# louiskirsch/speechT

Hardware: AMD Instinct MI355X
Metric: utterances/sec (training step, 10 s@16 kHz, batch 32) (higher is better)
Workload: dtype f32

## Files before the change

speecht_amd/csrc/api.hip:

```cpp
#include <algorithm>
#include <atomic>
#include <mutex>
#include <string>
#include <vector>
#include <string.h>

#include "st_common.h"

namespace st {
static thread_local char g_err[512] = "";
void set_error(const char* fmt, ...) {
  va_list ap;
  va_start(ap, fmt);
  vsnprintf(g_err, sizeof(g_err), fmt, ap);
  va_end(ap);
}

static std::atomic<int> g_trace_on{0};
static std::mutex g_trace_mu;
static std::vector<std::string> g_lines;
constexpr int kMaxTimed = 1 << 14;
struct TimedLaunch { int line; hipEvent_t e0, e1; };
static std::vector<TimedLaunch> g_timed;
static thread_local int g_last_line = -1;
static std::string g_timed_filter;
bool trace_on() { return g_trace_on.load(std::memory_order_relaxed) != 0; }
void trace(const char* fmt, ...) {
  if (!trace_on()) return;
  char line[320];
  va_list ap;
  va_start(ap, fmt);
  vsnprintf(line, sizeof(line), fmt, ap);
  va_end(ap);
  std::lock_guard<std::mutex> lock(g_trace_mu);
  if (g_lines.size() < (1u << 16)) {
    g_last_line = (int)g_lines.size();
    g_lines.emplace_back(line);
  } else {
    g_last_line = -1;
  }
}
LaunchTimer::LaunchTimer(hipStream_t) : start_(nullptr), stop_(nullptr) {
  const int line = g_last_line;
  g_last_line = -1;
  if (g_trace_on.load(std::memory_order_relaxed) != 2 || line < 0) return;
  hipEvent_t e0 = nullptr, e1 = nullptr;
  if (hipEventCreate(&e0) != hipSuccess) return;
  if (hipEventCreate(&e1) != hipSuccess) { hipEventDestroy(e0); return; }
  std::lock_guard<std::mutex> lock(g_trace_mu);
  if ((int)g_timed.size() >= kMaxTimed || line >= (int)g_lines.size() ||
      (!g_timed_filter.empty() && g_lines[line].find(g_timed_filter) == std::string::npos)) {
    hipEventDestroy(e0);
    hipEventDestroy(e1);
    return;
  }
  g_timed.push_back(TimedLaunch{line, e0, e1});
  start_ = e0;
  stop_ = e1;
}

static const char* const kTuneNames[TUNE_COUNT] = {"streamk", "streamk_slots", "streamk_test_drop", "no_fused_transforms",
                                                   "bf16_lag_copies", "filters_idft_valu", "bf16_taps_panel", "no_g3", "g3_tile"};
static std::atomic<int> g_tune[TUNE_COUNT];
int tuning(int key) { return g_tune[key].load(std::memory_order_relaxed); }
}

extern "C" {
int st_version(void) { return 200; }
const char* st_last_error(void) { return st::g_err; }

static int trace_begin(int mode) {
  std::lock_guard<std::mutex> lock(st::g_trace_mu);
  st::g_lines.clear();
  for (auto& t : st::g_timed) { hipEventDestroy(t.e0); hipEventDestroy(t.e1); }
  st::g_timed.clear();
  st::g_last_line = -1;
  st::g_trace_on.store(mode);
  return ST_OK;
}
int st_trace_begin(void) { return trace_begin(1); }
int st_trace_begin_timed(void) { return trace_begin(2); }
int st_trace_timed_filter(const char* text) {
  std::lock_guard<std::mutex> lock(st::g_trace_mu);
  st::g_timed_filter = text ? text : "";
  return ST_OK;
}

size_t st_trace_end(char* host_buf, size_t capacity) {
  st::g_trace_on.store(0);
  std::lock_guard<std::mutex> lock(st::g_trace_mu);
  for (auto& t : st::g_timed) {
    float ms = -1.f;
    if (hipEventSynchronize(t.e1) != hipSuccess || hipEventElapsedTime(&ms, t.e0, t.e1) != hipSuccess) ms = -1.f;
    char tail[48];
    snprintf(tail, sizeof(tail), " ms=%.5f", ms);
    if (t.line >= 0 && t.line < (int)st::g_lines.size()) st::g_lines[t.line] += tail;
    hipEventDestroy(t.e0);
    hipEventDestroy(t.e1);
  }
  st::g_timed.clear();
  size_t need = 1;
  for (const auto& l : st::g_lines) need += l.size() + 1;
  if (host_buf && capacity > 0) {
    size_t at = 0;
    for (const auto& l : st::g_lines) {
      if (at + l.size() + 1 >= capacity) break;
      memcpy(host_buf + at, l.data(), l.size());
      at += l.size();
      host_buf[at++] = '\n';
    }
    host_buf[at] = 0;
  }
  return need;
}

uint32_t st_host_crc32c(const void* host_data, size_t n, uint32_t crc) {
  static uint32_t table[8][256];
  static std::once_flag once;
  std::call_once(once, [] {
    for (uint32_t i = 0; i < 256; ++i) {
      uint32_t c = i;
      for (int k = 0; k < 8; ++k) c = (c >> 1) ^ (0x82F63B78u & (0u - (c & 1u)));
      table[0][i] = c;
    }
    for (uint32_t i = 0; i < 256; ++i)
      for (int t = 1; t < 8; ++t) table[t][i] = (table[t - 1][i] >> 8) ^ table[0][table[t - 1][i] & 0xFF];
  });
  const unsigned char* p = reinterpret_cast<const unsigned char*>(host_data);
  crc = ~crc;
  while (n >= 8) {
    uint32_t lo, hi;
    memcpy(&lo, p, 4);
    memcpy(&hi, p + 4, 4);
    lo ^= crc;
    crc = table[7][lo & 0xFF] ^ table[6][(lo >> 8) & 0xFF] ^ table[5][(lo >> 16) & 0xFF] ^ table[4][lo >> 24] ^
          table[3][hi & 0xFF] ^ table[2][(hi >> 8) & 0xFF] ^ table[1][(hi >> 16) & 0xFF] ^ table[0][hi >> 24];
    p += 8;
    n -= 8;
  }
  while (n--) crc = (crc >> 8) ^ table[0][(crc ^ *p++) & 0xFF];
  return ~crc;
}

int st_set_tuning(const char* name, int value) {
  ST_REQUIRE(name, "st_set_tuning: null name");
// ... 10 lines not shown
```

speecht_amd/csrc/conv_gemm.hip:

```cpp
#include <algorithm>
#include <atomic>
#include <cmath>
#include <cstdlib>

#include <type_traits>

#include "st_common.h"
#include "streamk_map.h"

namespace {

typedef float f32x16 __attribute__((ext_vector_type(16)));
typedef float f32x4 __attribute__((ext_vector_type(4)));

constexpr int BK = 32;
constexpr int APITCH = BK + 4;
constexpr int NTHREADS = 256;

struct RowMap {
  int frames;
  int row_stride;
  long batch_stride;
  long row0;
  __device__ __forceinline__ long off(int m) const {
    int b = m / frames;
    int t = m - b * frames;
    return (long)b * batch_stride + row0 + (long)t * row_stride;
  }
};

struct NNParams {
  const float* A;  RowMap amap;
  const float* Bm; int Np;
  float* C;        RowMap cmap;
  const float* mask; RowMap mmap;
  const float* bias;
  int M, Kvalid, Kp, n_store, relu;
  int taps, cp;
  int tiles_m, tiles_n, chunk;
  int gm, tm_per, tn_per;
  int splits, steps_per_split;
  float* slab;
  float* colsum;
  int colsum_rows;
  int batches;
  long a_batch, b_batch, c_batch;
  long bt_ld; int bt_rows;
};


__device__ __forceinline__ void dma16_sv(unsigned lds_byte_addr, const void* sbase, unsigned voff_bytes) {
  unsigned keep;
  asm volatile("s_mov_b32 %0, m0\n\ts_mov_b32 m0, %1\n\ts_nop 0\n\tglobal_load_lds_dwordx4 %2, %3\n\ts_mov_b32 m0, %0"
               : "=&s"(keep) : "s"(lds_byte_addr), "v"(voff_bytes), "s"(sbase) : "memory");
}
__device__ __forceinline__ float* at_bytes(float* ubase, unsigned voff_bytes) {
  return reinterpret_cast<float*>(reinterpret_cast<char*>(ubase) + voff_bytes);
}
__device__ __forceinline__ const float* at_bytes(const float* ubase, unsigned voff_bytes) {
  return reinterpret_cast<const float*>(reinterpret_cast<const char*>(ubase) + voff_bytes);
}
__device__ __forceinline__ void dma_wait_all() { asm volatile("s_waitcnt vmcnt(0)" ::: "memory"); }
__device__ __forceinline__ unsigned lds_addr(const float* p) {
  return (unsigned)(size_t)(__attribute__((address_space(3))) const float*)p;
}

template <int N> struct FVec;
template <> struct FVec<1> { typedef float type; };
template <> struct FVec<2> { typedef float type __attribute__((ext_vector_type(2))); };
template <> struct FVec<4> { typedef float type __attribute__((ext_vector_type(4))); };
template <int N> __device__ __forceinline__ float vget(const typename FVec<N>::type& v, int i) { return v[i]; }
template <> __device__ __forceinline__ float vget<1>(const float& v, int) { return v; }
template <int N> __device__ __forceinline__ void vset(typename FVec<N>::type& v, int i, float x) { v[i] = x; }
template <> __device__ __forceinline__ void vset<1>(float& v, int, float x) { v = x; }

__device__ __forceinline__ int swz_slot4(int lane, int row) { return ((lane & 7) ^ ((row >> 1) & 7)) * 4; }
__device__ __forceinline__ int swz_frag(int row, int q, int h) { return row * BK + (((2 * q + h) ^ ((row >> 1) & 7)) * 4); }

template <int BM, int BN, int WMW, int WNW, bool BT>
struct NNStage {
  static constexpr int WTM = BM / WMW, WTN = BN / WNW;
  static constexpr int MT = WTM / 32, NT = WTN / 32;
  static constexpr int A_DMA = BM / 32;
  static constexpr int B_DMA = BN / 32;
  static constexpr int N_DMA = A_DMA + B_DMA;
  static constexpr int A_SZ = BM * BK, B_SZ = BK * BN;
  typedef typename FVec<NT>::type bvec;

  template <int CUR, bool MORE, typename Dma, typename... Next>
  static __device__ __forceinline__ void run(const float* As, const float* Bs, const int (&a_frag)[4], const int (&bt_frag)[4],
                                             int b_frag, f32x16 (&acc)[MT][NT], int nq, Dma& dma_piece, Next... next) {
    const float* as = As + CUR * A_SZ;
    const float* bs = Bs + CUR * B_SZ + (BT ? 0 : b_frag);
    f32x4 af[4][MT];
    bvec bf[4][4];
    f32x4 bft[4][NT];
    auto read_frags = [&](int q) {
#pragma unroll
      for (int i = 0; i < MT; ++i) af[q][i] = *reinterpret_cast<const f32x4*>(as + a_frag[q] + i * 32 * BK);
      if (BT) {
#pragma unroll
        for (int n = 0; n < NT; ++n) bft[q][n] = *reinterpret_cast<const f32x4*>(bs + bt_frag[q] + n * 32 * BK);
      } else {
#pragma unroll
        for (int j = 0; j < 4; ++j) bf[q][j] = *reinterpret_cast<const bvec*>(bs + (8 * q + j) * BN);
      }
    };
    read_frags(0);
#pragma unroll
    for (int q = 0; q < 4; ++q) {
      if (MORE) {
#pragma unroll
        for (int pc = q; pc < N_DMA; pc += 4) dma_piece(pc, next..., CUR ^ 1);
      }
      if (q < 3) read_frags(q + 1);
      if (q < nq) {
#pragma unroll
        for (int j = 0; j < 4; ++j)
#pragma unroll
          for (int i = 0; i < MT; ++i)
#pragma unroll
            for (int n = 0; n < NT; ++n)
              acc[i][n] = __builtin_amdgcn_mfma_f32_32x32x2f32(af[q][i][j], BT ? bft[q][n][j] : vget<NT>(bf[q][j], n), acc[i][n], 0, 0, 0);
      }
#pragma unroll
      for (int k = 0; k < 4; ++k) {
        __builtin_amdgcn_sched_group_barrier(0x008, 1, 0);
        __builtin_amdgcn_sched_group_barrier(0x100, 1, 0);
      }
#pragma unroll
      for (int k = 0; k < 2; ++k) {
        __builtin_amdgcn_sched_group_barrier(0x008, 2, 0);
        __builtin_amdgcn_sched_group_barrier(0x006, 8, 0);
        __builtin_amdgcn_sched_group_barrier(0x010, 1, 0);
      }
      __builtin_amdgcn_sched_group_barrier(0x008, 8, 0);
      __builtin_amdgcn_sched_barrier(0);
// ... 556 lines not shown
    const int row = wn * WTN + l31;
#pragma unroll
    for (int q = 0; q < 4; ++q) bt_frag[q] = swz_frag(row, q, h);
  }
  const int b_frag = (4 * h) * BN + wn * WTN + NT * l31;

  f32x16 acc[MT][NT] = {}, acc2[MT][NT];

#pragma unroll
  for (int pcx = 0; pcx < N_DMA; ++pcx) dma_piece(pcx, p.a_off[0], p.b_off[0], 0);
  __syncthreads();

  auto stage = [&](auto cur_c, auto more_c, f32x16 (&tgt)[MT][NT], long nao, long nbo) __attribute__((always_inline)) {
    S::template run<decltype(cur_c)::value, decltype(more_c)::value>(As, Bs, a_frag, bt_frag, b_frag, tgt, 4, dma_piece, nao, nbo);
  };
  using std::integral_constant;
  using std::true_type;
  using std::false_type;
  const int spp = p.K / BK;
  auto phase = [&](f32x16 (&tgt)[MT][NT], long ao, long bo, long next_ao, long next_bo, auto last_c) __attribute__((always_inline)) {
    constexpr bool LAST = decltype(last_c)::value;
    for (int kt = 0; kt + 2 < spp; kt += 2) {
      stage(integral_constant<int, 0>{}, true_type{}, tgt, ao + (kt + 1) * BK, bo + (kt + 1) * bstep);
      stage(integral_constant<int, 1>{}, true_type{}, tgt, ao + (kt + 2) * BK, bo + (kt + 2) * bstep);
    }
    stage(integral_constant<int, 0>{}, true_type{}, tgt, ao + (spp - 1) * BK, bo + (spp - 1) * bstep);
    if (LAST) stage(integral_constant<int, 1>{}, false_type{}, tgt, 0L, 0L);
    else stage(integral_constant<int, 1>{}, true_type{}, tgt, next_ao, next_bo);
  };
  phase(acc, p.a_off[0], p.b_off[0], p.a_off[1], p.b_off[1], false_type{});
#pragma unroll
  for (int i = 0; i < MT; ++i)
#pragma unroll
    for (int j = 0; j < NT; ++j) acc2[i][j] = acc[i][j];
  phase(acc, p.a_off[1], p.b_off[1], p.a_off[2], p.b_off[2], false_type{});
  phase(acc2, p.a_off[2], p.b_off[2], 0L, 0L, true_type{});

  float* __restrict__ Cb = p.C + (long)bin * p.c_batch + n0 + wn * WTN + (BT ? l31 : NT * l31);
#pragma unroll
  for (int i = 0; i < MT; ++i)
#pragma unroll
    for (int r = 0; r < 16; ++r) {
      const int m = m0 + wm * WTM + i * 32 + (r & 3) + 8 * (r >> 2) + 4 * h;
      if (m < p.M) {
        float* row = Cb + (long)m * p.ldc;
        if (p.ksplit > 1) {
#pragma unroll
          for (int n = 0; n < NT; ++n) {
            const int cn = BT ? n * 32 : n;
            __hip_atomic_fetch_add(row + cn, acc[i][n][r], __ATOMIC_RELAXED, __HIP_MEMORY_SCOPE_AGENT);
            __hip_atomic_fetch_add(row + p.c_off2 + cn, acc2[i][n][r], __ATOMIC_RELAXED, __HIP_MEMORY_SCOPE_AGENT);
          }
        } else if (BT) {
#pragma unroll
          for (int n = 0; n < NT; ++n) { row[n * 32] = acc[i][n][r]; row[p.c_off2 + n * 32] = acc2[i][n][r]; }
        } else {
          bvec o1, o2;
#pragma unroll
          for (int n = 0; n < NT; ++n) { vset<NT>(o1, n, acc[i][n][r]); vset<NT>(o2, n, acc2[i][n][r]); }
          *reinterpret_cast<bvec*>(row) = o1;
          *reinterpret_cast<bvec*>(row + p.c_off2) = o2;
        }
      }
    }
}

struct TNParams {
  const float* A; RowMap amap;
  const float* Z; RowMap zmap;
  float* out;
  int M, Kvalid, Kp, Np, z_cols;
  int rows_per_split;
  int tiles_k, tiles_n;
  int amap_batches;
  int adv_b, adv_t;
  long a_batch, z_batch, o_batch;
  int z_shift;
};

__device__ __attribute__((aligned(16))) float g_zero_row[4] = {0.f, 0.f, 0.f, 0.f};

constexpr int TN_THREADS = NTHREADS;

template <int BN, int WKW, int WNW>
__global__ __launch_bounds__(TN_THREADS) void gemm_tn_kernel(TNParams p) {
  constexpr int BKO = 128;
  constexpr int BMR = 32;
  constexpr int WTK = BKO / WKW, WTN = BN / WNW;
  constexpr int MT = WTK / 32, NT = WTN / 32;
  constexpr int A_DMA = BKO / 32, Z_DMA = BN / 32;
  constexpr int A_LPR = BKO / 4, Z_LPR = BN / 4;
  constexpr int A_SZ = BMR * BKO, Z_SZ = BMR * BN;
  constexpr int N_DMA = A_DMA + Z_DMA;
  static_assert(WKW * WNW == 4 && (MT == 1 || MT == 2 || MT == 4) && (NT == 1 || NT == 2 || NT == 4), "tile config");
  typedef typename FVec<MT>::type avec;
  typedef typename FVec<NT>::type zvec;

  __shared__ __attribute__((aligned(16))) float smem[2 * A_SZ + 2 * Z_SZ];
  float* const As = smem;
  float* const Zs = smem + 2 * A_SZ;

  int tile_k, tile_n;
  {
    const int bid = blockIdx.x;
    const int total = p.tiles_k * p.tiles_n;
    if ((p.tiles_k & 7) == 0 && (p.tiles_n & 7) == 0) {
      const int idx = (bid & 7) * (total >> 3) + (bid >> 3);
      const int sb = idx >> 6, within = idx & 63;
      const int sbn = p.tiles_n >> 3;
      tile_k = (sb / sbn) * 8 + (within >> 3);
      tile_n = (sb % sbn) * 8 + (within & 7);
    } else {
      tile_n = bid % p.tiles_n;
      tile_k = bid / p.tiles_n;
    }
  }
  const int k0 = tile_k * BKO, n0 = tile_n * BN;
  const int split = blockIdx.y;
  const float* __restrict__ Ab = p.A + (long)blockIdx.z * p.a_batch;
  const float* __restrict__ Zb = p.Z + (long)(blockIdx.z >> p.z_shift) * p.z_batch;
  const int m_begin = split * p.rows_per_split;
  const int m_end = min(p.M, m_begin + p.rows_per_split);

  const int tid = threadIdx.x;
  const int lane = tid & 63;
  const int wave = __builtin_amdgcn_readfirstlane(tid >> 6);
  const int l31 = lane & 31, h = lane >> 5;
  const int wk = wave / WNW, wn = wave % WNW;

  f32x16 acc[MT][NT] = {};

  const int nstages = (m_end - m_begin + BMR - 1) / BMR;

  constexpr int A_PIECES = BMR * A_LPR / 64, Z_PIECES = BMR * Z_LPR / 64;
  constexpr int A_PW = (A_PIECES + 3) / 4, Z_PW = (Z_PIECES + 3) / 4;
  const int acol = min(k0 + (lane % A_LPR) * 4, p.Kvalid - 4);
  const int zcol = min(n0 + (lane % Z_LPR) * 4, p.z_cols - 4);
  const int arow = lane / A_LPR, zrow = lane / Z_LPR;
  const long a_jump = p.amap.batch_stride - (long)p.amap.frames * p.amap.row_stride;
  const long z_jump = p.zmap.batch_stride - (long)p.zmap.frames * p.zmap.row_stride;
  const bool tiny = p.amap.frames < BMR;
  const unsigned a_voff = (unsigned)((arow * p.amap.row_stride + acol) * 4);
  const unsigned z_voff = (unsigned)((zrow * p.zmap.row_stride + zcol) * 4);
  const unsigned lds_a = lds_addr(As), lds_z = lds_addr(Zs);
  const long a_step = (long)(64 / A_LPR) * p.amap.row_stride * 4, z_step = (long)(64 / Z_LPR) * p.zmap.row_stride * 4;
  int sb = min(m_begin, p.M - 1) / p.amap.frames;
  int stt = min(m_begin, p.M - 1) - sb * p.amap.frames;

  auto issue_slice = [&](int sl, int mb, int buf) {
    const bool plain = !tiny && stt + BMR <= p.amap.frames && mb + BMR <= m_end;
    if (plain) {
      const char* sa = reinterpret_cast<const char*>(Ab + ((long)sb * p.amap.batch_stride + p.amap.row0 + (long)stt * p.amap.row_stride));
      const char* sz = reinterpret_cast<const char*>(Zb + ((long)sb * p.zmap.batch_stride + p.zmap.row0 + (long)stt * p.zmap.row_stride));
#pragma unroll
      for (int i = sl; i < A_PW; i += 4) {
        const int pc = wave * A_PW + i;
        if (pc < A_PIECES) dma16_sv(lds_a + (buf * A_SZ + pc * 256) * 4, sa + pc * a_step, a_voff);
      }
#pragma unroll
      for (int i = sl; i < Z_PW; i += 4) {
        const int pc = wave * Z_PW + i;
        if (pc < Z_PIECES) dma16_sv(lds_z + (buf * Z_SZ + pc * 256) * 4, sz + pc * z_step, z_voff);
      }
    } else {
#pragma unroll
      for (int i = sl; i < A_PW + Z_PW; i += 4) {
        const bool isA = i < A_PW;
        const int pc = isA ? wave * A_PW + i : wave * Z_PW + (i - A_PW);
        if (pc >= (isA ? A_PIECES : Z_PIECES)) continue;
        const int r = isA ? pc * (64 / A_LPR) + arow : pc * (64 / Z_LPR) + zrow;
        const int m = min(mb + r, p.M - 1);
        const float* g = isA ? Ab + p.amap.off(m) + acol : Zb + p.zmap.off(m) + zcol;
        if (mb + r >= m_end) g = g_zero_row;
        float* dst = isA ? As + buf * A_SZ + pc * 256 : Zs + buf * Z_SZ + pc * 256;
        __builtin_amdgcn_global_load_lds((st::gptr_t)g, (st::lptr_t)dst, 16, 0, 0);
      }
    }
  };
  auto stage_advance = [&]() {
    stt += p.adv_t; sb += p.adv_b;
    if (stt >= p.amap.frames) { stt -= p.amap.frames; ++sb; }
  };

  if (nstages > 0) {
#pragma unroll
    for (int sl = 0; sl < 4; ++sl) issue_slice(sl, m_begin, 0);
    stage_advance();
  }
  dma_wait_all();
  __syncthreads();

  const int a_frag = (4 * h) * BKO + wk * WTK + MT * l31;
  const int z_frag = (4 * h) * BN + wn * WTN + NT * l31;
  for (int st = 0; st < nstages; ++st) {
    const int cur = st & 1;
    const bool more = st + 1 < nstages;
    const int mb_next = m_begin + (st + 1) * BMR;
    const float* as = As + cur * A_SZ + a_frag;
    const float* zs = Zs + cur * Z_SZ + z_frag;
    avec af[4][4];
    zvec zf[4][4];
    auto read_frags = [&](int q) {
#pragma unroll
      for (int j = 0; j < 4; ++j) {
        af[q][j] = *reinterpret_cast<const avec*>(as + (8 * q + j) * BKO);
        zf[q][j] = *reinterpret_cast<const zvec*>(zs + (8 * q + j) * BN);
      }
    };
    read_frags(0);
#pragma unroll
    for (int q = 0; q < 4; ++q) {
      if (more) issue_slice(q, mb_next, cur ^ 1);
      if (q < 3) read_frags(q + 1);
#pragma unroll
      for (int j = 0; j < 4; ++j)
#pragma unroll
        for (int i = 0; i < MT; ++i)
#pragma unroll
          for (int n = 0; n < NT; ++n)
            acc[i][n] = __builtin_amdgcn_mfma_f32_32x32x2f32(vget<MT>(af[q][j], i), vget<NT>(zf[q][j], n), acc[i][n], 0, 0, 0);
#pragma unroll
      for (int k = 0; k < 8; ++k) {
        __builtin_amdgcn_sched_group_barrier(0x008, 1, 0);
        __builtin_amdgcn_sched_group_barrier(0x100, 1, 0);
      }
      __builtin_amdgcn_sched_group_barrier(0x008, 8, 0);
      __builtin_amdgcn_sched_barrier(0);
    }
    if (more) stage_advance();
    dma_wait_all();
    __syncthreads();
  }

  float* out = p.out + (long)split * p.Kp * p.Np + (long)blockIdx.z * p.o_batch;
  const int col0 = n0 + wn * WTN + NT * l31;
#pragma unroll
  for (int i = 0; i < MT; ++i)
#pragma unroll
    for (int r = 0; r < 16; ++r) {
      const int k = k0 + wk * WTK + MT * ((r & 3) + 8 * (r >> 2) + 4 * h) + i;
      if (k < p.Kp && col0 < p.Np) {
        zvec o;
#pragma unroll
        for (int n = 0; n < NT; ++n)
          vset<NT>(o, n, (k < p.Kvalid && col0 + n < p.z_cols) ? acc[i][n][r] : 0.f);
        *reinterpret_cast<zvec*>(out + (long)k * p.Np + col0) = o;
      }
    }
}

struct TN3Params {
  const float* A; long lda, a_batch; long a_off[3];
  const float* Z; long ldz, z_batch; long z_off[3];
  float* out; long o_batch, o_part;
  int M, K, N, tiles_k, tiles_n, batches;
};

__global__ __launch_bounds__(TN_THREADS, 2) void gemm_tn_g3_kernel(TN3Params p) {
  constexpr int BKO = 128, BN = 128, BMR = 32, WKW = 2, WNW = 2;
  constexpr int WTK = BKO / WKW, WTN = BN / WNW;
  constexpr int MT = WTK / 32, NT = WTN / 32;
  constexpr int A_LPR = BKO / 4, Z_LPR = BN / 4;
  constexpr int A_SZ = BMR * BKO, Z_SZ = BMR * BN;
  constexpr int A_PIECES = BMR * A_LPR / 64, Z_PIECES = BMR * Z_LPR / 64;
  constexpr int A_PW = A_PIECES / 4, Z_PW = Z_PIECES / 4;
  typedef typename FVec<MT>::type avec;
  typedef typename FVec<NT>::type zvec;
  __shared__ __attribute__((aligned(16))) float smem[2 * A_SZ + 2 * Z_SZ];
  float* const As = smem;
  float* const Zs = smem + 2 * A_SZ;

  int bin, tile_k, tile_n;
  if (!bin_tile(p.tiles_k, p.tiles_n, p.batches, bin, tile_k, tile_n)) return;
  const int k0 = tile_k * BKO, n0 = tile_n * BN;

  const int tid = threadIdx.x;
  const int lane = tid & 63;
  const int wave = __builtin_amdgcn_readfirstlane(tid >> 6);
  const int l31 = lane & 31, h = lane >> 5;
  const int wk = wave / WNW, wn = wave % WNW;

  const char* Ab = reinterpret_cast<const char*>(p.A + (long)bin * p.a_batch + k0);
  const char* Zb = reinterpret_cast<const char*>(p.Z + (long)bin * p.z_batch + n0);
  const unsigned a_voff = (unsigned)(((lane / A_LPR) * p.lda + (lane % A_LPR) * 4) * 4);
  const unsigned z_voff = (unsigned)(((lane / Z_LPR) * p.ldz + (lane % Z_LPR) * 4) * 4);
  const unsigned lds_a = lds_addr(As), lds_z = lds_addr(Zs);
  const long a_step = (long)(64 / A_LPR) * p.lda * 4, z_step = (long)(64 / Z_LPR) * p.ldz * 4;
  const long a_stage = (long)BMR * p.lda * 4, z_stage = (long)BMR * p.ldz * 4;

  auto issue_slice = [&](int sl, const char* sa, const char* sz, int buf) {
#pragma unroll
    for (int i = sl; i < A_PW; i += 4) {
      const int pc = wave * A_PW + i;
      dma16_sv(lds_a + (buf * A_SZ + pc * 256) * 4, sa + pc * a_step, a_voff);
    }
#pragma unroll
    for (int i = sl; i < Z_PW; i += 4) {
      const int pc = wave * Z_PW + i;
      dma16_sv(lds_z + (buf * Z_SZ + pc * 256) * 4, sz + pc * z_step, z_voff);
    }
  };

  f32x16 acc[MT][NT], acc2[MT][NT];
#pragma unroll
  for (int i = 0; i < MT; ++i)
#pragma unroll
    for (int j = 0; j < NT; ++j)
#pragma unroll
      for (int r = 0; r < 16; ++r) acc[i][j][r] = 0.f;

  const int spp = p.M / BMR;
  const int a_frag = (4 * h) * BKO + wk * WTK + MT * l31;
  const int z_frag = (4 * h) * BN + wn * WTN + NT * l31;
  int gst = 0;
// ... 340 lines not shown
    const double per_cu = (double)tiles / 256.0;
    const bool uneven = tiles > 256 && tiles <= 768 && std::ceil(per_cu) / per_cu > 1.2;
    int slots = st::tuning(st::TUNE_STREAMK_SLOTS);
    if (slots != 64 && slots != 96) slots = 64;
    st::SkPlan plan;
    if ((knob == 1 || uneven) && tiles < (1L << 24) && st::sk_make_plan((int)tiles, K / BK, slots, plan)) {
      static std::atomic<unsigned> g_epoch{0};
      unsigned epoch = g_epoch.fetch_add(1, std::memory_order_relaxed) + 1;
      if (epoch == 0) epoch = g_epoch.fetch_add(1, std::memory_order_relaxed) + 1;
      BinsParams q{};
      q.A = A; q.B = B; q.C = C;
      q.lda = lda; q.ldb = b_transposed ? K : N; q.ldc = ldc;
      q.a_batch = a_batch; q.b_batch = b_batch; q.c_batch = c_batch;
      q.tiles_m = M / 64; q.tiles_n = N / 128;
      q.plan = plan;
      q.ctrl = reinterpret_cast<unsigned*>(sk_ws);
      q.partial = sk_ws + st::SK_CTRL_WORDS;
      q.epoch = epoch;
      q.pub_epoch = st::tuning(st::TUNE_STREAMK_TEST_DROP) ? (epoch ^ 0x80000000u) : epoch;
      st::trace("gemm_nn_bins<64,128,2,2%s> batched bins=%d M=%d Np=%d Kp=%d streamk wgs=%d upw=%d gflop=%.3f", b_transposed ? ",bt" : "",
                batches, M, N, K, 8 * plan.wgs_per_xcd, plan.upw, 2e-9 * M * (double)N * K * batches);
      {
        st::LaunchTimer timer(s);
        const dim3 grid(8 * plan.wgs_per_xcd), block(NTHREADS);
        if (b_transposed) st::launch_timed(timer, gemm_nn_bins_kernel<64, 128, 2, 2, true>, grid, block, s, q);
        else st::launch_timed(timer, gemm_nn_bins_kernel<64, 128, 2, 2, false>, grid, block, s, q);
      }
      return st::check_launch("gemm_nn_bins");
    }
  }
  if (M % 128 == 64 && M > 128 && (long)K * N >= (1L << 21) && (long)st::ceil_div(M, 128) * (N / 128) * batches >= 512) {
    if (int e = st::gemm_nn_batched(A, lda, a_batch, B, b_batch, C, ldc, c_batch, M - 64, K, N, batches, s, nullptr, b_transposed)) return e;
    return st::gemm_nn_batched(A + (long)(M - 64) * lda, lda, a_batch, B, b_batch, C + (long)(M - 64) * ldc, ldc, c_batch, 64, K, N, batches, s,
                               nullptr, b_transposed);
  }
  NNParams p{};
  p.A = A;
  p.amap.frames = M; p.amap.row_stride = (int)lda; p.amap.batch_stride = 0; p.amap.row0 = 0;
  p.Bm = B;
  p.Np = N;
  p.C = C;
  p.cmap.frames = M; p.cmap.row_stride = (int)ldc; p.cmap.batch_stride = 0; p.cmap.row0 = 0;
  p.M = M;
  p.Kvalid = K;
  p.Kp = K;
  p.n_store = N;
  p.taps = 1;
  p.cp = K;
  p.batches = batches;
  p.a_batch = a_batch; p.b_batch = b_batch; p.c_batch = c_batch;
  if (b_transposed) { p.bt_ld = K; p.bt_rows = N; }
  return run_nn(p, 0, s);
}

int st::gemm_tn_batched(const float* A, long lda, long a_batch, const float* Z, long ldz, long z_batch, float* out,
                        long o_batch, int M, int K, int N, int batches, hipStream_t s, int z_batch_shift, int tile_n) {
  if (!(A && Z && out && M > 0 && M % 32 == 0 && K % 128 == 0 && N % 128 == 0 && batches > 0 && (tile_n == 0 || tile_n == 64 || tile_n == 128))) {
    st::set_error("gemm_tn_batched: bad shape M=%d K=%d N=%d tile_n=%d", M, K, N, tile_n);
    return ST_EINVAL;
  }
  if (tile_n == 0) {
    const long tiles128 = (long)batches * (K / 128) * (N / 128);
    tile_n = (tiles128 > 256 && tiles128 <= 320 && M <= 512) ? 64 : 128;
  }
  TNParams p{};
  p.A = A;
  p.amap.frames = M; p.amap.row_stride = (int)lda; p.amap.batch_stride = 0; p.amap.row0 = 0;
  p.Z = Z;
  p.zmap.frames = M; p.zmap.row_stride = (int)ldz; p.zmap.batch_stride = 0; p.zmap.row0 = 0;
  p.M = M;
  p.Kvalid = K;
  p.Kp = K;
  p.Np = N;
  p.z_cols = N;
  p.rows_per_split = M;
  p.out = out;
  p.tiles_k = K / 128;
  p.tiles_n = N / tile_n;
  p.amap_batches = 1;
  p.adv_b = 32 / M;
  p.adv_t = 32 % M;
  p.a_batch = a_batch; p.z_batch = z_batch; p.o_batch = o_batch;
  p.z_shift = z_batch_shift;
  st::trace("gemm_tn<%d> batched bins=%d M=%d Kp=%d Np=%d gflop=%.3f", tile_n, batches, M, K, N, 2e-9 * M * (double)K * N * batches);
  {
    st::LaunchTimer timer(s);
    const dim3 grid(p.tiles_k * p.tiles_n, 1, batches);
    if (tile_n == 64) st::launch_timed(timer, gemm_tn_kernel<64, 2, 2>, grid, dim3(TN_THREADS), s, p);
    else st::launch_timed(timer, gemm_tn_kernel<128, 2, 2>, grid, dim3(TN_THREADS), s, p);
  }
  return st::check_launch("gemm_tn_batched");
}

int st::gemm_nn_g3_batched(const float* A, long lda, long a_batch, const long a_off[3], const float* B, long ldb, long b_batch,
                           const long b_off[3], float* C, long ldc, long c_batch, long c_off2, int M, int K, int N, int batches,
                           hipStream_t s, bool b_transposed) {
  if (!(A && B && C && M > 0 && K > 0 && K % 64 == 0 && N % 128 == 0 && batches > 0 && lda % 4 == 0 && ldb % 4 == 0 && ldc % 4 == 0 &&
        c_off2 % 4 == 0 && a_off[0] % 4 == 0 && a_off[1] % 4 == 0 && a_off[2] % 4 == 0 && b_off[0] % 4 == 0 && b_off[1] % 4 == 0 && b_off[2] % 4 == 0)) {
    st::set_error("gemm_nn_g3_batched: bad shape M=%d K=%d N=%d", M, K, N);
    return ST_EINVAL;
  }
  if (M % 128 == 64 && M > 128 && (long)batches * st::ceil_div(M, 128) * (N / 128) >= 512 &&
      st::tuning(st::TUNE_G3_TILE) == 0) {
    if (int e = st::gemm_nn_g3_batched(A, lda, a_batch, a_off, B, ldb, b_batch, b_off, C, ldc, c_batch, c_off2, M - 64, K, N, batches, s, b_transposed)) return e;
    return st::gemm_nn_g3_batched(A + (long)(M - 64) * lda, lda, a_batch, a_off, B, ldb, b_batch, b_off, C + (long)(M - 64) * ldc, ldc, c_batch, c_off2,
                                  64, K, N, batches, s, b_transposed);
  }
  G3Params p{};
  p.A = A; p.lda = lda; p.a_batch = a_batch;
  p.B = B; p.ldb = ldb; p.b_batch = b_batch;
  for (int i = 0; i < 3; ++i) { p.a_off[i] = a_off[i]; p.b_off[i] = b_off[i]; }
  p.C = C; p.ldc = ldc; p.c_batch = c_batch; p.c_off2 = c_off2;
  p.M = M; p.N = N; p.batches = batches;
  const long wgs128 = (long)batches * st::ceil_div(M, 128) * (N / 128), wgs64 = (long)batches * st::ceil_div(M, 64) * (N / 128);
  const int tile = st::tuning(st::TUNE_G3_TILE);
  const bool half_rows = tile == 2 ? false : (tile == 1 || tile == 4 || M <= 64 || wgs128 < 512);
  p.ksplit = (half_rows && K % 128 == 0 && (tile == 4 || (tile == 0 && wgs64 < 512))) ? 2 : 1;
  p.K = K / p.ksplit;
  p.tiles_m = st::ceil_div(M, half_rows ? 64 : 128);
  p.tiles_n = N / 128;
  if (p.ksplit > 1)
    hipLaunchKernelGGL(g3_zero_out_kernel, dim3(st::ceil_div(M, 4), batches), dim3(256), 0, s, C, ldc, c_batch, c_off2, M, N);
  const dim3 grid(st::ceil_div(batches, 8) * p.tiles_m * p.tiles_n * 8, p.ksplit), block(NTHREADS);
  st::trace("gemm_nn_g3<%d%s> batched bins=%d M=%d Np=%d Kp=%d ksplit=%d gflop=%.3f", half_rows ? 64 : 128, b_transposed ? ",bt" : "", batches, M, N, K,
            p.ksplit, 2e-9 * p.tiles_m * (half_rows ? 64 : 128) * (double)N * 3 * K * batches);
  st::LaunchTimer timer(s);
  if (half_rows) {
    if (b_transposed) st::launch_timed(timer, gemm_nn_g3_kernel<64, true>, grid, block, s, p);
    else st::launch_timed(timer, gemm_nn_g3_kernel<64, false>, grid, block, s, p);
  } else {
    if (b_transposed) st::launch_timed(timer, gemm_nn_g3_kernel<128, true>, grid, block, s, p);
    else st::launch_timed(timer, gemm_nn_g3_kernel<128, false>, grid, block, s, p);
  }
  return st::check_launch("gemm_nn_g3");
}

int st::gemm_tn_g3_batched(const float* A, long lda, long a_batch, const long a_off[3], const float* Z, long ldz, long z_batch,
                           const long z_off[3], float* out, long o_batch, long o_part, int M, int K, int N, int batches, hipStream_t s) {
  if (!(A && Z && out && M > 0 && M % 32 == 0 && K % 128 == 0 && N % 128 == 0 && batches > 0 && lda % 4 == 0 && ldz % 4 == 0 &&
        (long)32 * lda < (1L << 29) && (long)32 * ldz < (1L << 29))) {
    st::set_error("gemm_tn_g3_batched: bad shape M=%d K=%d N=%d", M, K, N);
    return ST_EINVAL;
  }
  TN3Params p{};
  p.A = A; p.lda = lda; p.a_batch = a_batch;
  p.Z = Z; p.ldz = ldz; p.z_batch = z_batch;
  for (int i = 0; i < 3; ++i) { p.a_off[i] = a_off[i]; p.z_off[i] = z_off[i]; }
  p.out = out; p.o_batch = o_batch; p.o_part = o_part;
  p.M = M; p.K = K; p.N = N; p.tiles_k = K / 128; p.tiles_n = N / 128; p.batches = batches;
  st::trace("gemm_tn_g3<128> batched bins=%d M=%d Kp=%d Np=%d gflop=%.3f", batches, M, K, N, 2e-9 * 3 * M * (double)K * N * batches);
  st::LaunchTimer timer(s);
  st::launch_timed(timer, gemm_tn_g3_kernel, dim3(st::ceil_div(batches, 8) * p.tiles_k * p.tiles_n * 8), dim3(TN_THREADS), s, p);
  return st::check_launch("gemm_tn_g3_batched");
}

static int bwd_data_impl(const st_tensor3* dz, const float* packed_t, bool forward_filters, int width, int pad_left,
                         const st_tensor3* act, const st_tensor3* dx, float* dbias_dx, void* workspace,
                         size_t workspace_bytes, void* stream);

extern "C" {

int st_streamk_lost_ptr(void** device_word) {
  ST_REQUIRE(device_word, "st_streamk_lost_ptr: null argument");
  void* p = nullptr;
  if (hipGetSymbolAddress(&p, HIP_SYMBOL(g_sk_lost)) != hipSuccess || !p) {
    st::set_error("st_streamk_lost_ptr: hipGetSymbolAddress failed");
    return ST_ELAUNCH;
  }
  *device_word = p;
  return ST_OK;
}
// ... 352 lines not shown
```

speecht_amd/csrc/st_common.h:

```cpp
#pragma once
#include <hip/hip_runtime.h>
#include <hip/hip_ext.h>
#include <stdarg.h>
#include <stdio.h>

#include "speecht_hip.h"

namespace st {

void set_error(const char* fmt, ...);

bool trace_on();
void trace(const char* fmt, ...);
class LaunchTimer {
 public:
  explicit LaunchTimer(hipStream_t s);
  bool active() const { return start_ != nullptr; }
  hipEvent_t start() const { return start_; }
  hipEvent_t stop() const { return stop_; }

 private:
  hipEvent_t start_, stop_;
};
template <typename... KArgs, typename... Args>
inline void launch_timed(const LaunchTimer& t, void (*kernel)(KArgs...), const dim3& grid, const dim3& block, hipStream_t s,
                         Args&&... args) {
  static_assert(sizeof...(KArgs) == sizeof...(Args), "launch_timed: argument count does not match the kernel");
  if (t.active()) hipExtLaunchKernelGGL(kernel, grid, block, 0, s, t.start(), t.stop(), 0, static_cast<KArgs>(args)...);
  else hipLaunchKernelGGL(kernel, grid, block, 0, s, static_cast<KArgs>(args)...);
}
enum { TUNE_STREAMK, TUNE_STREAMK_SLOTS, TUNE_STREAMK_TEST_DROP, TUNE_NO_FUSED_TRANSFORMS, TUNE_BF16_LAG_COPIES, TUNE_FILTERS_IDFT_VALU,
       TUNE_BF16_TAPS_PANEL, TUNE_NO_G3, TUNE_G3_TILE, TUNE_COUNT };
int tuning(int key);

constexpr int SK_FLAGS = 0, SK_TIMEOUTS = 768, SK_CTRL_WORDS = 1024;
constexpr long SK_WS_FLOATS = SK_CTRL_WORDS + 768L * 64 * 128;
int gemm_nn_batched(const float* A, long lda, long a_batch, const float* B, long b_batch, float* C, long ldc, long c_batch,
                    int M, int K, int N, int batches, hipStream_t s, float* sk_ws = nullptr, bool b_transposed = false);
int gemm_tn_batched(const float* A, long lda, long a_batch, const float* Z, long ldz, long z_batch, float* out, long o_batch,
                    int M, int K, int N, int batches, hipStream_t s, int z_batch_shift = 0, int tile_n = 0);
int gemm_nn_g3_batched(const float* A, long lda, long a_batch, const long a_off[3], const float* B, long ldb, long b_batch,
                       const long b_off[3], float* C, long ldc, long c_batch, long c_off2, int M, int K, int N, int batches,
                       hipStream_t s, bool b_transposed = false);
int gemm_tn_g3_batched(const float* A, long lda, long a_batch, const long a_off[3], const float* Z, long ldz, long z_batch,
                       const long z_off[3], float* out, long o_batch, long o_part, int M, int K, int N, int batches, hipStream_t s);

int gemm_bf16_bins(int planes, const void* a_planes, size_t a_plane, long a_rows_apart, long a_bin, const void* bt_planes,
                   size_t b_plane, long ldb, long b_bin, float* c, long ldc, int rows, int k, int n, int bins, hipStream_t s,
                   int b_bin_shift = 0);
int lag_products_tr_bf16(const void* s_plane, const void* z_plane, int bins, int rows, int half, int npo, float* q, hipStream_t s);
bool conv_taps_bf16_eligible(const st_tensor3& a, const st_tensor3& y, int width, int lead, const st_tensor3* act);
int conv_taps_bf16(const st_tensor3& a, const void* a_plane, const void* filters, const float* bias, int width, int lead, int relu,
                   const st_tensor3* act, const void* act_plane, const st_tensor3& y, void* y_plane, hipStream_t s);
int transpose_bf16_bins(const void* src, void* dst, int bins, int rows, int cols, hipStream_t s);
int transpose_bf16_bins_split(const void* src, void* dst, int bins, int rows, int cols, int forms, hipStream_t s);

inline hipStream_t as_stream(void* s) { return reinterpret_cast<hipStream_t>(s); }

inline int check_launch(const char* what) {
  hipError_t e = hipGetLastError();
  if (e != hipSuccess) {
    set_error("%s: %s", what, hipGetErrorString(e));
    return ST_ELAUNCH;
  }
  return ST_OK;
}

#define ST_REQUIRE(cond, ...)      \
  do {                             \
    if (!(cond)) {                 \
      st::set_error(__VA_ARGS__);  \
      return ST_EINVAL;            \
    }                              \
  } while (0)

inline int ceil_div(int a, int b) { return (a + b - 1) / b; }
inline size_t round_up(size_t a, size_t b) { return (a + b - 1) / b * b; }

inline int npad_of(int cout) { return cout <= 32 ? 32 : (cout <= 64 ? 64 : (int)round_up(cout, 128)); }

inline bool tensor_ok(const st_tensor3* t) {
  return t && t->base && t->batch > 0 && t->frames > 0 && t->channels > 0 && t->halo >= 0 && t->c_pitch % 16 == 0 &&
         t->c_pitch >= t->channels && t->t_pitch >= t->halo + t->frames;
}

inline long row_offset(const st_tensor3& x, int b, int t) {
  return ((long)b * x.t_pitch + x.halo + t) * (long)x.c_pitch;
}

typedef __attribute__((address_space(1))) const void* gptr_t;
typedef __attribute__((address_space(3))) void* lptr_t;

__device__ __forceinline__ float wave_sum(float v) {
#pragma unroll
  for (int o = 32; o > 0; o >>= 1) v += __shfl_xor(v, o, 64);
  return v;
}
__device__ __forceinline__ float wave_max(float v) {
#pragma unroll
  for (int o = 32; o > 0; o >>= 1) v = fmaxf(v, __shfl_xor(v, o, 64));
  return v;
}

}
```

Measured before the change: 4938.

## Add four-slot DMA ring pipeline to gemm_tn kernel for small-M tiles

Adds an optional four-deep LDS ring buffer to the transposed GEMM kernel. Each stage becomes 16 rows instead of 32, and loads are issued several stages ahead, with partial vmcnt waits taking the place of a full drain before each barrier. A host policy turns the ring on by default for tile_n=64 with at most 512 rows, and a tuning knob can force it on or off. The intent is to hide global-to-LDS latency in short-M reductions, at the cost of more stages, more barriers and smaller per-stage MFMA work.

After: 4937. No clear change (-0.0%).

```diff
diff --git a/speecht_amd/csrc/api.hip b/speecht_amd/csrc/api.hip
--- a/speecht_amd/csrc/api.hip
+++ b/speecht_amd/csrc/api.hip
@@ -60,7 +60,7 @@
 }
 
 static const char* const kTuneNames[TUNE_COUNT] = {"streamk", "streamk_slots", "streamk_test_drop", "no_fused_transforms",
-                                                   "bf16_lag_copies", "filters_idft_valu", "bf16_taps_panel", "no_g3", "g3_tile"};
+                                                   "bf16_lag_copies", "filters_idft_valu", "bf16_taps_panel", "no_g3", "g3_tile", "tn_ring"};
 static std::atomic<int> g_tune[TUNE_COUNT];
 int tuning(int key) { return g_tune[key].load(std::memory_order_relaxed); }
 }
diff --git a/speecht_amd/csrc/conv_gemm.hip b/speecht_amd/csrc/conv_gemm.hip
--- a/speecht_amd/csrc/conv_gemm.hip
+++ b/speecht_amd/csrc/conv_gemm.hip
@@ -7,6 +7,7 @@
 
 #include "st_common.h"
 #include "streamk_map.h"
+#include "tn_ring.h"
 
 namespace {
 
@@ -53,6 +54,11 @@
   unsigned keep;
   asm volatile("s_mov_b32 %0, m0\n\ts_mov_b32 m0, %1\n\ts_nop 0\n\tglobal_load_lds_dwordx4 %2, %3\n\ts_mov_b32 m0, %0"
                : "=&s"(keep) : "s"(lds_byte_addr), "v"(voff_bytes), "s"(sbase) : "memory");
+}
+__device__ __forceinline__ void dma16_vv(unsigned lds_byte_addr, const void* lane_ptr) {
+  unsigned keep;
+  asm volatile("s_mov_b32 %0, m0\n\ts_mov_b32 m0, %1\n\ts_nop 0\n\tglobal_load_lds_dwordx4 %2, off\n\ts_mov_b32 m0, %0"
+               : "=&s"(keep) : "s"(lds_byte_addr), "v"(lane_ptr) : "memory");
 }
 __device__ __forceinline__ float* at_bytes(float* ubase, unsigned voff_bytes) {
   return reinterpret_cast<float*>(reinterpret_cast<char*>(ubase) + voff_bytes);
@@ -775,10 +781,12 @@
 
 constexpr int TN_THREADS = NTHREADS;
 
-template <int BN, int WKW, int WNW>
+template <int BN, int WKW, int WNW, int RING = 2>
 __global__ __launch_bounds__(TN_THREADS) void gemm_tn_kernel(TNParams p) {
   constexpr int BKO = 128;
-  constexpr int BMR = 32;
+  constexpr int BMR = st::TN_RING_ROWS / RING;
+  constexpr int NSL = BMR / 8;
+  static_assert(RING == 2 || RING == 4, "ring depth");
   constexpr int WTK = BKO / WKW, WTN = BN / WNW;
   constexpr int MT = WTK / 32, NT = WTN / 32;
   constexpr int A_DMA = BKO / 32, Z_DMA = BN / 32;
@@ -789,9 +797,9 @@
   typedef typename FVec<MT>::type avec;
   typedef typename FVec<NT>::type zvec;
 
-  __shared__ __attribute__((aligned(16))) float smem[2 * A_SZ + 2 * Z_SZ];
+  __shared__ __attribute__((aligned(16))) float smem[RING * A_SZ + RING * Z_SZ];
   float* const As = smem;
-  float* const Zs = smem + 2 * A_SZ;
+  float* const Zs = smem + RING * A_SZ;
 
   int tile_k, tile_n;
   {
@@ -823,7 +831,7 @@
 
   f32x16 acc[MT][NT] = {};
 
-  const int nstages = (m_end - m_begin + BMR - 1) / BMR;
+  const int nstages = RING == 2 ? (m_end - m_begin + BMR - 1) / BMR : (m_end > m_begin ? st::tn_ring_stages(m_end - m_begin, RING) : 0);
 
   constexpr int A_PIECES = BMR * A_LPR / 64, Z_PIECES = BMR * Z_LPR / 64;
   constexpr int A_PW = (A_PIECES + 3) / 4, Z_PW = (Z_PIECES + 3) / 4;
@@ -846,18 +854,18 @@
       const char* sa = reinterpret_cast<const char*>(Ab + ((long)sb * p.amap.batch_stride + p.amap.row0 + (long)stt * p.amap.row_stride));
       const char* sz = reinterpret_cast<const char*>(Zb + ((long)sb * p.zmap.batch_stride + p.zmap.row0 + (long)stt * p.zmap.row_stride));
 #pragma unroll
-      for (int i = sl; i < A_PW; i += 4) {
+      for (int i = sl; i < A_PW; i += NSL) {
         const int pc = wave * A_PW + i;
         if (pc < A_PIECES) dma16_sv(lds_a + (buf * A_SZ + pc * 256) * 4, sa + pc * a_step, a_voff);
       }
 #pragma unroll
-      for (int i = sl; i < Z_PW; i += 4) {
+      for (int i = sl; i < Z_PW; i += NSL) {
         const int pc = wave * Z_PW + i;
         if (pc < Z_PIECES) dma16_sv(lds_z + (buf * Z_SZ + pc * 256) * 4, sz + pc * z_step, z_voff);
       }
     } else {
 #pragma unroll
-      for (int i = sl; i < A_PW + Z_PW; i += 4) {
+      for (int i = sl; i < A_PW + Z_PW; i += NSL) {
         const bool isA = i < A_PW;
         const int pc = isA ? wave * A_PW + i : wave * Z_PW + (i - A_PW);
         if (pc >= (isA ? A_PIECES : Z_PIECES)) continue;
@@ -866,33 +874,55 @@
         const float* g = isA ? Ab + p.amap.off(m) + acol : Zb + p.zmap.off(m) + zcol;
         if (mb + r >= m_end) g = g_zero_row;
         float* dst = isA ? As + buf * A_SZ + pc * 256 : Zs + buf * Z_SZ + pc * 256;
-        __builtin_amdgcn_global_load_lds((st::gptr_t)g, (st::lptr_t)dst, 16, 0, 0);
+        if (RING == 2) __builtin_amdgcn_global_load_lds((st::gptr_t)g, (st::lptr_t)dst, 16, 0, 0);
+        else dma16_vv(isA ? lds_a + (buf * A_SZ + pc * 256) * 4 : lds_z + (buf * Z_SZ + pc * 256) * 4, g);
       }
     }
   };
+  const int ring_adv_b = RING == 2 ? 0 : BMR / p.amap.frames, ring_adv_t = RING == 2 ? 0 : BMR % p.amap.frames;
   auto stage_advance = [&]() {
-    stt += p.adv_t; sb += p.adv_b;
+    stt += RING == 2 ? p.adv_t : ring_adv_t; sb += RING == 2 ? p.adv_b : ring_adv_b;
     if (stt >= p.amap.frames) { stt -= p.amap.frames; ++sb; }
   };
 
-  if (nstages > 0) {
-#pragma unroll
-    for (int sl = 0; sl < 4; ++sl) issue_slice(sl, m_begin, 0);
-    stage_advance();
-  }
-  dma_wait_all();
-  __syncthreads();
+  constexpr int LPS = A_PW + Z_PW;
+  static_assert(RING == 2 || (A_PIECES % 4 == 0 && Z_PIECES % 4 == 0), "ring: every wave issues the same number of loads per stage");
+  auto ring_wait = [&](int st) {
+    const int pending = st::tn_ring_pending(st, nstages, RING);
+    if (pending >= 2) asm volatile("s_waitcnt vmcnt(%0)\n\ts_barrier" ::"n"(2 * LPS) : "memory");
+    else if (pending == 1) asm volatile("s_waitcnt vmcnt(%0)\n\ts_barrier" ::"n"(LPS) : "memory");
+    else asm volatile("s_waitcnt vmcnt(0)\n\ts_barrier" ::: "memory");
+  };
+  if (RING == 2) {
+    if (nstages > 0) {
+#pragma unroll
+      for (int sl = 0; sl < NSL; ++sl) issue_slice(sl, m_begin, 0);
+      stage_advance();
+    }
+    dma_wait_all();
+  } else {
+    const int pro = st::tn_ring_prologue(nstages, RING);
+    for (int s = 0; s < pro; ++s) {
+#pragma unroll
+      for (int sl = 0; sl < NSL; ++sl) issue_slice(sl, m_begin + s * BMR, st::tn_ring_slot(s, RING));
+      stage_advance();
+    }
+    ring_wait(-1);
+  }
+  if (RING == 2) __syncthreads();
 
   const int a_frag = (4 * h) * BKO + wk * WTK + MT * l31;
   const int z_frag = (4 * h) * BN + wn * WTN + NT * l31;
   for (int st = 0; st < nstages; ++st) {
-    const int cur = st & 1;
-    const bool more = st + 1 < nstages;
-    const int mb_next = m_begin + (st + 1) * BMR;
+    const int nxt = RING == 2 ? (st + 1 < nstages ? st + 1 : -1) : st::tn_ring_issue(st, nstages, RING);
+    const int cur = RING == 2 ? (st & 1) : st::tn_ring_slot(st, RING);
+    const int nbuf = RING == 2 ? (cur ^ 1) : st::tn_ring_slot(nxt, RING);
+    const bool more = RING == 2 ? st + 1 < nstages : nxt >= 0;
+    const int mb_next = m_begin + (RING == 2 ? st + 1 : nxt) * BMR;
     const float* as = As + cur * A_SZ + a_frag;
     const float* zs = Zs + cur * Z_SZ + z_frag;
-    avec af[4][4];
-    zvec zf[4][4];
+    avec af[NSL][4];
+    zvec zf[NSL][4];
     auto read_frags = [&](int q) {
 #pragma unroll
       for (int j = 0; j < 4; ++j) {
@@ -902,9 +932,9 @@
     };
     read_frags(0);
 #pragma unroll
-    for (int q = 0; q < 4; ++q) {
-      if (more) issue_slice(q, mb_next, cur ^ 1);
-      if (q < 3) read_frags(q + 1);
+    for (int q = 0; q < NSL; ++q) {
+      if (more) issue_slice(q, mb_next, nbuf);
+      if (q < NSL - 1) read_frags(q + 1);
 #pragma unroll
       for (int j = 0; j < 4; ++j)
 #pragma unroll
@@ -921,8 +951,8 @@
       __builtin_amdgcn_sched_barrier(0);
     }
     if (more) stage_advance();
-    dma_wait_all();
-    __syncthreads();
+    if (RING == 2) { dma_wait_all(); __syncthreads(); }
+    else ring_wait(st);
   }
 
   float* out = p.out + (long)split * p.Kp * p.Np + (long)blockIdx.z * p.o_batch;
@@ -1429,11 +1459,14 @@
   p.adv_t = 32 % M;
   p.a_batch = a_batch; p.z_batch = z_batch; p.o_batch = o_batch;
   p.z_shift = z_batch_shift;
-  st::trace("gemm_tn<%d> batched bins=%d M=%d Kp=%d Np=%d gflop=%.3f", tile_n, batches, M, K, N, 2e-9 * M * (double)K * N * batches);
+  const int ring = st::tn_ring_policy(M, tile_n, st::tuning(st::TUNE_TN_RING));
+  st::trace("gemm_tn<%d> batched bins=%d M=%d Kp=%d Np=%d gflop=%.3f ring=%d", tile_n, batches, M, K, N, 2e-9 * M * (double)K * N * batches, ring);
   {
     st::LaunchTimer timer(s);
     const dim3 grid(p.tiles_k * p.tiles_n, 1, batches);
-    if (tile_n == 64) st::launch_timed(timer, gemm_tn_kernel<64, 2, 2>, grid, dim3(TN_THREADS), s, p);
+    if (tile_n == 64 && ring == 4) st::launch_timed(timer, gemm_tn_kernel<64, 2, 2, 4>, grid, dim3(TN_THREADS), s, p);
+    else if (tile_n == 64) st::launch_timed(timer, gemm_tn_kernel<64, 2, 2>, grid, dim3(TN_THREADS), s, p);
+    else if (ring == 4) st::launch_timed(timer, gemm_tn_kernel<128, 2, 2, 4>, grid, dim3(TN_THREADS), s, p);
     else st::launch_timed(timer, gemm_tn_kernel<128, 2, 2>, grid, dim3(TN_THREADS), s, p);
   }
   return st::check_launch("gemm_tn_batched");
diff --git a/speecht_amd/csrc/st_common.h b/speecht_amd/csrc/st_common.h
--- a/speecht_amd/csrc/st_common.h
+++ b/speecht_amd/csrc/st_common.h
@@ -30,7 +30,7 @@
   else hipLaunchKernelGGL(kernel, grid, block, 0, s, static_cast<KArgs>(args)...);
 }
 enum { TUNE_STREAMK, TUNE_STREAMK_SLOTS, TUNE_STREAMK_TEST_DROP, TUNE_NO_FUSED_TRANSFORMS, TUNE_BF16_LAG_COPIES, TUNE_FILTERS_IDFT_VALU,
-       TUNE_BF16_TAPS_PANEL, TUNE_NO_G3, TUNE_G3_TILE, TUNE_COUNT };
+       TUNE_BF16_TAPS_PANEL, TUNE_NO_G3, TUNE_G3_TILE, TUNE_TN_RING, TUNE_COUNT };
 int tuning(int key);
 
 constexpr int SK_FLAGS = 0, SK_TIMEOUTS = 768, SK_CTRL_WORDS = 1024;
diff --git a/speecht_amd/csrc/tn_ring.h b/speecht_amd/csrc/tn_ring.h
--- /dev/null
+++ b/speecht_amd/csrc/tn_ring.h
@@ -0,0 +1,33 @@
+#pragma once
+
+#ifdef __HIPCC__
+#define ST_RING_HD __host__ __device__ inline __attribute__((always_inline))
+#else
+#define ST_RING_HD inline
+#endif
+
+namespace st {
+
+constexpr int TN_RING_ROWS = 64;
+constexpr int TN_RING_PAD = 32;
+
+ST_RING_HD int tn_ring_depth(int slots) { return TN_RING_ROWS / slots; }
+ST_RING_HD int tn_ring_stages(int rows, int slots) {
+  return (rows + TN_RING_PAD - 1) / TN_RING_PAD * (TN_RING_PAD / tn_ring_depth(slots));
+}
+ST_RING_HD int tn_ring_slot(int stage, int slots) { return stage % slots; }
+ST_RING_HD int tn_ring_prologue(int nstages, int slots) { return nstages < slots - 1 ? nstages : slots - 1; }
+ST_RING_HD int tn_ring_issue(int st, int nstages, int slots) { return st + slots - 1 < nstages ? st + slots - 1 : -1; }
+ST_RING_HD int tn_ring_pending(int st, int nstages, int slots) {
+  int ahead = nstages - 1 - st;
+  if (ahead > slots - 1) ahead = slots - 1;
+  return ahead > 0 ? ahead - 1 : 0;
+}
+
+constexpr int TN_RING_MAX_ROWS = 512;
+inline int tn_ring_policy(int rows, int tile_n, int knob) {
+  if (knob == 1 || (tile_n != 64 && tile_n != 128)) return 2;
+  return (knob == 2 || (tile_n == 64 && rows <= TN_RING_MAX_ROWS)) ? 4 : 2;
+}
+
+}
```
